# bkomuves/zikkurat-algebra

Hardware: AMD Instinct MI355X
Metric: BLS12-381 G1 MSM pairs/sec at 2^20; Fr NTT 2^24 elems/sec (1/2/4/8 GPU) (higher is better)
Workload: dtype u32-limb Montgomery Fp (381-bit)

## Files before the change

include/zkalgebra_gpu.h:

```cpp
#ifndef ZKALGEBRA_GPU_H
#define ZKALGEBRA_GPU_H

#include <stddef.h>
#include <stdint.h>

#ifdef __cplusplus
extern "C" {
#endif

#define ZKG_API __attribute__((visibility("default")))


ZKG_API void bn128_G1_proj_MSM_mont_coeff_proj_out(int npoints, const uint64_t *expos, const uint64_t *grps, uint64_t *tgt, int expo_nlimbs);
ZKG_API void bn128_G1_proj_MSM_std_coeff_proj_out(int npoints, const uint64_t *expos, const uint64_t *grps, uint64_t *tgt, int expo_nlimbs);
ZKG_API void bn128_G1_proj_MSM_mont_coeff_affine_out(int npoints, const uint64_t *expos, const uint64_t *grps, uint64_t *tgt, int expo_nlimbs);
ZKG_API void bn128_G1_proj_MSM_std_coeff_affine_out(int npoints, const uint64_t *expos, const uint64_t *grps, uint64_t *tgt, int expo_nlimbs);
ZKG_API void bn128_G1_proj_MSM_std_coeff_proj_out_variable(int npoints, const uint64_t *expos, const uint64_t *grps, uint64_t *tgt, int expo_nlimbs, int window_size);

ZKG_API void bls12_381_G1_proj_MSM_mont_coeff_proj_out(int npoints, const uint64_t *expos, const uint64_t *grps, uint64_t *tgt, int expo_nlimbs);
ZKG_API void bls12_381_G1_proj_MSM_std_coeff_proj_out(int npoints, const uint64_t *expos, const uint64_t *grps, uint64_t *tgt, int expo_nlimbs);
ZKG_API void bls12_381_G1_proj_MSM_mont_coeff_affine_out(int npoints, const uint64_t *expos, const uint64_t *grps, uint64_t *tgt, int expo_nlimbs);
ZKG_API void bls12_381_G1_proj_MSM_std_coeff_affine_out(int npoints, const uint64_t *expos, const uint64_t *grps, uint64_t *tgt, int expo_nlimbs);
ZKG_API void bls12_381_G1_proj_MSM_std_coeff_proj_out_variable(int npoints, const uint64_t *expos, const uint64_t *grps, uint64_t *tgt, int expo_nlimbs, int window_size);

// ... 271 lines not shown
                                     const uint64_t *base_affine, int affine_out, uint64_t *d_tgt);
ZKG_API int zkg_g2_scl_powers(int curve, int n, const uint64_t *a, const uint64_t *tau, const uint64_t *base_affine,
                              int affine_out, uint64_t *tgt);
ZKG_API void zkg_g2_scl_set_window(int c);
ZKG_API void zkg_g2_scl_set_fixed_min(int n);
ZKG_API int  zkg_g2_scl_last_path(void);
ZKG_API size_t zkg_g2_scl_table_bytes(int curve, int c);

ZKG_API void zkg_g1_proj_add(int curve, const uint64_t *a, const uint64_t *b, uint64_t *out);
ZKG_API void zkg_g1_proj_normalize(int curve, const uint64_t *a, uint64_t *out);
ZKG_API void zkg_g1_proj_to_affine(int curve, const uint64_t *a, uint64_t *out);

ZKG_API void zkg_gen_fr(int curve, uint64_t seed, int64_t start, int64_t count, uint64_t *out);
ZKG_API void zkg_gen_g1_points(int curve, uint64_t seed, int64_t start, int64_t count, uint64_t *out);
ZKG_API void zkg_fft_generator(int curve, int m, uint64_t *out);

ZKG_API int zkg_msm_default_window(int npoints);
ZKG_API int zkg_msm_window(int curve, int npoints, int expo_nlimbs, int expos_mont);

ZKG_API void zkg_msm_profile(int on);
ZKG_API void zkg_msm_set_group_limit(size_t entries);
ZKG_API void zkg_msm_set_ysum_mode(int mode);
ZKG_API void zkg_msm_set_ahead_min(int lg);
ZKG_API void zkg_ntt_set_max_radix(int r);
ZKG_API void zkg_ntt_set_table_max(size_t entries);
ZKG_API void zkg_ntt_ext_set_max_grid(unsigned tiles);
ZKG_API void zkg_ntt_set_cache_limit(size_t bytes);
ZKG_API size_t zkg_ntt_cache_bytes(void);
ZKG_API void zkg_arena_set_limit(size_t bytes);
ZKG_API int zkg_msm_last_groups(void);
ZKG_API int zkg_g1_fft_last_glv(void);
ZKG_API int zkg_g1_fft_plan(int curve, int m, int *bits, int cap);
ZKG_API int zkg_g1_fft_radix_products(int b);
ZKG_API size_t zkg_msm_workspace_bytes(int curve, int npoints, int expo_nlimbs, int expos_mont, int host_inputs,
                                       int window_size, int groups);

ZKG_API void bn128_pairing_affine(const uint64_t *P, const uint64_t *Q, uint64_t *tgt);
ZKG_API void bn128_pairing_projective(const uint64_t *P, const uint64_t *Q, uint64_t *tgt);
ZKG_API void bls12_381_pairing_affine(const uint64_t *P, const uint64_t *Q, uint64_t *tgt);
ZKG_API void bls12_381_pairing_projective(const uint64_t *P, const uint64_t *Q, uint64_t *tgt);
ZKG_API int zkg_pairing_rows(int curve, int n, const uint64_t *P, const uint64_t *Q, uint64_t *tgt);
ZKG_API int zkg_pairing_rows_device(int curve, int n, const uint64_t *d_P, const uint64_t *d_Q, uint64_t *d_tgt);
ZKG_API int zkg_pairing_product(int curve, int n, const uint64_t *P, const uint64_t *Q, uint64_t *tgt);
ZKG_API int zkg_pairing_product_device(int curve, int n, const uint64_t *d_P, const uint64_t *d_Q, uint64_t *d_tgt);
ZKG_API int zkg_pairing_final_expo(int curve, int n, const uint64_t *src, uint64_t *tgt);
ZKG_API int zkg_pairing_final_expo_device(int curve, int n, const uint64_t *d_src, uint64_t *d_tgt);
// ... 24 lines not shown
```

zikkurat-algebra_amd/csrc/zk_capi.cpp:

```cpp
#include <hip/hip_runtime.h>
#include <string.h>
#include "../../include/zkalgebra_gpu.h"
#include "zk_gen.hpp"
#include "zk_host.hpp"
#include "zk_msm.hpp"
#include "zk_ntt.hpp"
#include "zk_runtime.hpp"

using namespace zk;

namespace {

enum Out { PROJ, AFFINE, JAC };

template <class C>
void msm_entry(int npoints, const uint64_t *expos, const uint64_t *grps, uint64_t *tgt, int nl, bool mont,
               int window, Out out) {
  using HF = typename HostOf<C>::Fp;
  constexpr int NP = C::NP64;
  uint64_t proj[3 * NP];
  bool ok = false;
  guard([&] {
    msm_g1<C>(npoints, expos, nl, grps, true, mont, window, proj);
    ok = true;
// ... 318 lines not shown
    const uint64_t v[] = ZK_BN128_FFT_GEN_FR64;
    memcpy(g.v, v, sizeof g.v);
    for (int i = m; i < ZK_BN128_FFT_LOG; i++) zkh::sqr(g, g);
    memcpy(out, g.v, sizeof g.v);
  } else {
    zkh::Fe<zkh::BLS_Fr> g;
    const uint64_t v[] = ZK_BLS12_381_FFT_GEN_FR64;
    memcpy(g.v, v, sizeof g.v);
    for (int i = m; i < ZK_BLS12_381_FFT_LOG; i++) zkh::sqr(g, g);
    memcpy(out, g.v, sizeof g.v);
  }
}

ZKG_API int zkg_msm_default_window(int npoints) { return zk::msm_default_window(npoints); }
ZKG_API int zkg_msm_window(int curve, int npoints, int expo_nlimbs, int expos_mont) {
  const int bits = expos_mont ? (curve == ZKG_BN128 ? 254 : 255) : 64 * (expo_nlimbs < 4 ? expo_nlimbs : 4);
  return zk::msm_default_window_bits(npoints, bits);
}

ZKG_API void zkg_msm_profile(int on) { zk::msm_set_profile(on); }
ZKG_API void zkg_msm_set_group_limit(size_t entries) { zk::msm_set_group_limit(entries); }
ZKG_API void zkg_msm_set_ysum_mode(int mode) { zk::msm_set_ysum_mode(mode); }
ZKG_API void zkg_msm_set_ahead_min(int lg) { zk::msm_set_ahead_min(lg); }
ZKG_API void zkg_ntt_set_max_radix(int r) { zk::ntt_set_max_radix(r); }

ZKG_API void zkg_ntt_set_table_max(size_t entries) { zk::ntt_set_table_max(entries); }
ZKG_API void zkg_ntt_ext_set_max_grid(unsigned tiles) { zk::ntt_ext_set_max_grid(tiles); }
ZKG_API void zkg_ntt_set_cache_limit(size_t bytes) { zk::ntt_set_cache_limit(bytes); }
ZKG_API size_t zkg_ntt_cache_bytes(void) { return guard_ret<size_t>(0, [&] { return zk::ntt_cache_bytes(); }); }
ZKG_API void zkg_arena_set_limit(size_t bytes) { zk::arena_set_limit(bytes); }
ZKG_API int zkg_msm_last_groups(void) { return zk::msm_last_groups_read(); }
ZKG_API size_t zkg_msm_workspace_bytes(int curve, int npoints, int expo_nlimbs, int expos_mont, int host_inputs,
                                       int window_size, int groups) {
  return guard_ret<size_t>(0, [&] {
    if (curve == ZKG_BN128)
      return zk::msm_workspace_bytes<BN254>(npoints, expo_nlimbs, expos_mont != 0, host_inputs != 0, window_size,
                                            groups);
    return zk::msm_workspace_bytes<BLS381>(npoints, expo_nlimbs, expos_mont != 0, host_inputs != 0, window_size,
                                           groups);
  });
}

ZKG_API int zkg_set_devices(const int *ids, int n) { return zk::set_device_set(ids, n); }
ZKG_API int zkg_get_devices(int *ids, int cap) {
  const std::vector<int> v = zk::device_set();
  for (int i = 0; i < (int)v.size() && i < cap; i++) ids[i] = v[i];
// ... 24 lines not shown
```

zikkurat-algebra_amd/csrc/zk_msm.hip:

```cpp
#include "zk_msm_impl.hpp"

namespace zk {

int msm_default_window(int n) {
  if (n <= 1) return 4;
  const int lg = ilog2((unsigned)n);
  int c;
  if (lg <= 10) c = lg - 1;
  else if (lg <= 12) c = 10;
  else if (lg <= 16) c = 13;
  else if (lg <= 24) c = 16;
  else c = 20;
  if (c < 4) c = 4;
  if (c > 20) c = 20;
  return c;
}

int msm_default_window_bits(int n, int bits) {
  const int c = msm_default_window(n);
  if (n <= 1) return c;
  const int lg = ilog2((unsigned)n);
  if (bits == 254 && lg >= 20 && lg <= 24) return 17;
  if (bits == 255 && (lg == 23 || lg == 24)) return 20;
  return c;
}

void msm_set_ysum_mode(int mode) { ysum_mode().store(mode < 0 ? -1 : (mode ? 1 : 0)); }
void msm_set_ahead_min(int lg) { msm_ahead_min().store(lg < 0 ? -1 : lg); }
void msm_set_profile(int on) { msm_profile_flag().store(on); }
int msm_last_groups_read() { return msm_last_groups().load(); }
void msm_set_group_limit(size_t entries) {
  msm_group_limit().store(entries == 0 || entries > MSM_MAX_GROUP_ENTRIES ? MSM_MAX_GROUP_ENTRIES : entries);
}

template size_t msm_workspace_bytes<BN254>(int, int, bool, bool, int, int);
template size_t msm_workspace_bytes<BLS381>(int, int, bool, bool, int, int);
template void msm_g1<BN254>(int, const uint64_t *, int, const uint64_t *, bool, bool, int, uint64_t *);
template void msm_g1<BLS381>(int, const uint64_t *, int, const uint64_t *, bool, bool, int, uint64_t *);

}
```

zikkurat-algebra_amd/csrc/zk_msm.hpp:

```cpp
#pragma once
#include <stddef.h>
#include <stdint.h>
#include "zk_curve.hpp"
#include "zk_host.hpp"

namespace zk {

template <class C> struct HostOf;
template <> struct HostOf<BN254> {
  using Fp = zkh::BN_Fp;
  using Fr = zkh::BN_Fr;
  static void b3(zkh::Fe<Fp> &r) { const uint64_t v[] = ZK_BN128_B3_FP64; memcpy(r.v, v, sizeof r.v); }
};
template <> struct HostOf<BLS381> {
  using Fp = zkh::BLS_Fp;
  using Fr = zkh::BLS_Fr;
  static void b3(zkh::Fe<Fp> &r) { const uint64_t v[] = ZK_BLS12_381_B3_FP64; memcpy(r.v, v, sizeof r.v); }
};

template <> struct HostOf<BN254_G2> {
  using Fp = zkh::HF2<zkh::BN_Fp>;
  using Fr = zkh::BN_Fr;
};
template <> struct HostOf<BLS381_G2> {
  using Fp = zkh::HF2<zkh::BLS_Fp>;
  using Fr = zkh::BLS_Fr;
};

int msm_default_window(int n);
int msm_default_window_bits(int n, int bits);
void msm_set_profile(int on);
void msm_set_group_limit(size_t entries);
void msm_set_ysum_mode(int mode);
void msm_set_ahead_min(int lg);
int msm_last_groups_read();

template <class C>
size_t msm_workspace_bytes(int n, int nl, bool mont, bool host_inputs, int window, int groups);
template <class C>
void msm_g1(int n, const uint64_t *scalars, int nl, const uint64_t *points, bool host_inputs, bool mont,
            int window, uint64_t *out_proj);

}
```

zikkurat-algebra_amd/csrc/zk_msm_impl.hpp:

```cpp
#pragma once
#include <hipcub/hipcub.hpp>
#include <algorithm>
#include <atomic>
#include <chrono>
#include <memory>
#include <thread>
#include <vector>
#include "zk_curve.hpp"
#include "zk_quad.hpp"
#include "zk_host.hpp"
#include "zk_runtime.hpp"
#include "zk_msm.hpp"
#include "zk_ntt.hpp"

namespace zk {

template <class C>
__global__ void __launch_bounds__(256) k_points_int(const uint64_t *__restrict__ pts, int n,
                                                    uint32_t *__restrict__ out) {
  using F = typename C::Fp;
  constexpr int IN4 = 2 * F::N64 * 8 / 16;
  constexpr int OUT4 = aff_words<F>() / 4;
  constexpr int ST4 = IN4 > OUT4 ? IN4 : OUT4;
  __shared__ uint4 stage[256 * ST4];
// ... 85 lines not shown
constexpr int FINE_LDS_MAX = 8192;
constexpr int FINE_LDS_BYTES = 150 * 1024;
static int fine_stage_cap(int s) {
  const int cap = (FINE_LDS_BYTES - (4 << s)) / 4;
  return cap < FINE_LDS_MAX ? cap : FINE_LDS_MAX;
}

__device__ __forceinline__ uint32_t block_excl_scan256(uint32_t v, uint32_t *tmp, uint32_t *total) {
  const int t = threadIdx.x;
  tmp[t] = v;
  __syncthreads();
  for (int d = 1; d < 256; d <<= 1) {
    const uint32_t o = t >= d ? tmp[t - d] : 0;
    __syncthreads();
    tmp[t] += o;
    __syncthreads();
  }
  const uint32_t incl = tmp[t];
  *total = tmp[255];
  __syncthreads();
  return incl - v;
}

template <bool SCATTER>
__global__ void __launch_bounds__(256) k_coarse(const uint32_t *__restrict__ dig, int n, int plo, int phi, int M,
                                                int s, int nbins, uint32_t *__restrict__ cnt,
                                                uint32_t *__restrict__ tmpv, uint16_t *__restrict__ tmpf) {
  __shared__ uint32_t hist[MSM_COARSE_BINS], lofs[MSM_COARSE_BINS], gcur[MSM_COARSE_BINS], scan_tmp[256];
  __shared__ uint32_t sv[SORT_CHUNK], sk[SORT_CHUNK];
  const uint32_t w = blockIdx.y, g = blockIdx.x, nwg = gridDim.x;
  const int t = threadIdx.x;
  const int e0 = plo + (int)g * M, e1 = min(phi, e0 + M);
  const uint32_t *d = dig + (size_t)w * n;
  uint32_t *cw = cnt + (size_t)w * nbins * nwg + g;
  if (!SCATTER) {
    if (w == 0 && g == 0 && t == 0) cnt[(size_t)gridDim.y * nbins * nwg] = 0;
    for (int b = t; b < nbins; b += 256) hist[b] = 0;
    __syncthreads();
    for (int b0 = e0; b0 < e1; b0 += 256 * COUNT_ILP) {
      uint32_t mag[COUNT_ILP];
#pragma unroll
      for (int j = 0; j < COUNT_ILP; j++) {
        const int e = b0 + j * 256 + t;
        mag[j] = e < e1 ? d[e] & 0x7fffffffu : 0u;
      }
#pragma unroll
      for (int j = 0; j < COUNT_ILP; j++)
        if (mag[j]) atomicAdd(&hist[(mag[j] - 1) >> s], 1u);
    }
    __syncthreads();
    for (int b = t; b < nbins; b += 256) cw[(size_t)b * nwg] = hist[b];
    return;
  }
  for (int b = t; b < nbins; b += 256) gcur[b] = cw[(size_t)b * nwg];
  const uint32_t fmask = (1u << s) - 1;
  constexpr int PER = SORT_CHUNK / 256;
  for (int c0 = e0; c0 < e1; c0 += SORT_CHUNK) {
    for (int b = t; b < nbins; b += 256) hist[b] = 0;
    __syncthreads();
    uint32_t val[PER], key[PER], rank[PER];
#pragma unroll
    for (int k = 0; k < PER; k++) {
      const int e = c0 + k * 256 + t;
      const uint32_t v = e < e1 ? d[e] : 0u;
      const uint32_t mag = v & 0x7fffffffu;
      key[k] = 0xffffffffu;
      if (mag) {
        const uint32_t b = (mag - 1) >> s;
        key[k] = (b << 16) | ((mag - 1) & fmask);
        val[k] = (uint32_t)e | (v & 0x80000000u);
        rank[k] = atomicAdd(&hist[b], 1u);
      }
    }
    __syncthreads();
    uint32_t tot;
    const uint32_t h = t < nbins ? hist[t] : 0u;
    const uint32_t ex = block_excl_scan256(h, scan_tmp, &tot);
    if (t < nbins) lofs[t] = ex;
    __syncthreads();
#pragma unroll
    for (int k = 0; k < PER; k++) {
      if (key[k] != 0xffffffffu) {
        const uint32_t p = lofs[key[k] >> 16] + rank[k];
        sv[p] = val[k];
        sk[p] = key[k];
      }
    }
    __syncthreads();
    for (uint32_t i = t; i < tot; i += 256) {
      const uint32_t k = sk[i], b = k >> 16;
      const uint32_t slot = gcur[b] + (i - lofs[b]);
      tmpv[slot] = sv[i];
      tmpf[slot] = (uint16_t)(k & 0xffffu);
    }
    __syncthreads();
    if (t < nbins) gcur[t] += h;
  }
}

template <bool SCATTER>
// ... 85 lines not shown
    const int leader = __ffsll((unsigned long long)m) - 1;
    const uint32_t lk = (uint32_t)__builtin_amdgcn_readlane((int)key, leader);
    const bool mine = todo && key == lk;
    const uint64_t same = __ballot(mine);
    const int cnt = __popcll(same);
    if (cnt < 4) break;
    if (RET) {
      uint32_t base = 0;
      if ((int)lane == leader) base = atomicAdd(&ctr[lk], (uint32_t)cnt);
      base = (uint32_t)__builtin_amdgcn_readlane((int)base, leader);
      if (mine) r = base + (uint32_t)__popcll(same & below);
    } else if ((int)lane == leader) {
      atomicAdd(&ctr[lk], (uint32_t)cnt);
    }
    if (mine) todo = false;
  }
  if (todo) {
    if (RET) r = atomicAdd(&ctr[key], 1u);
    else atomicAdd(&ctr[key], 1u);
  }
  return r;
}

template <int BS>
__device__ __forceinline__ uint32_t block_excl_scan(uint32_t v, uint32_t *wtot, uint32_t *total) {
  const int t = threadIdx.x, lane = t & 63, w = t >> 6;
  uint32_t x = v;
#pragma unroll
  for (int d = 1; d < 64; d <<= 1) {
    const uint32_t o = (uint32_t)__shfl_up((int)x, d, 64);
    if (lane >= d) x += o;
  }
  if (lane == 63) wtot[w] = x;
  __syncthreads();
  uint32_t off = 0, all = 0;
#pragma unroll
  for (int k = 0; k < BS / 64; k++) {
    off += k < w ? wtot[k] : 0u;
    all += wtot[k];
  }
  *total = all;
  __syncthreads();
  return off + x - v;
}

template <int FINE_BS, int FINE_ILP, bool AGG>
static __global__ void __launch_bounds__(FINE_BS) k_fine(const uint32_t *__restrict__ coff, int nwg, uint32_t nq,
                                                         int s, int cap, const uint32_t *__restrict__ tmpv,
                                                         const uint16_t *__restrict__ tmpf,
                                                         uint32_t *__restrict__ list, uint32_t *__restrict__ offsets,
                                                         uint32_t base) {
  extern __shared__ uint32_t fh[];
  __shared__ uint32_t wtot[FINE_BS / 64];
  const int F = 1 << s, t = threadIdx.x;
  uint32_t *sv = fh + F;
  const uint32_t q = blockIdx.x;
  const uint32_t start = coff[(size_t)q * nwg];
  const uint32_t end = coff[(size_t)(q + 1) * nwg];
  const bool staged = end - start <= (uint32_t)cap;
  constexpr uint32_t STEP = FINE_BS * FINE_ILP;
  for (int f = t; f < F; f += FINE_BS) fh[f] = 0;
  __syncthreads();
  for (uint32_t e0 = start; e0 < end; e0 += STEP) {
    uint32_t k[FINE_ILP];
#pragma unroll
    for (int j = 0; j < FINE_ILP; j++) {
      const uint32_t e = e0 + j * FINE_BS + t;
      k[j] = e < end ? tmpf[e] : 0u;
    }
#pragma unroll
    for (int j = 0; j < FINE_ILP; j++) {
      const bool act = e0 + j * FINE_BS + t < end;
      if (AGG) lds_inc_agg<false>(fh, k[j], act);
      else if (act) atomicAdd(&fh[k[j]], 1u);
    }
  }
  __syncthreads();
  const int per = (F + FINE_BS - 1) / FINE_BS;
  uint32_t sum = 0;
  for (int j = 0; j < per; j++) {
    const int f = t * per + j;
    if (f < F) sum += fh[f];
  }
  uint32_t tot;
  uint32_t run = block_excl_scan<FINE_BS>(sum, wtot, &tot);
  for (int j = 0; j < per; j++) {
    const int f = t * per + j;
    if (f < F) {
      const uint32_t h = fh[f];
      fh[f] = staged ? run : start + run;
      offsets[(size_t)q * F + f] = base + start + run;
      run += h;
    }
  }
  if (q == nq - 1 && t == 0) offsets[(size_t)nq * F] = base + end;
  __syncthreads();
  for (uint32_t e0 = start; e0 < end; e0 += STEP) {
    uint32_t k[FINE_ILP], v[FINE_ILP];
#pragma unroll
    for (int j = 0; j < FINE_ILP; j++) {
      const uint32_t e = e0 + j * FINE_BS + t;
      k[j] = e < end ? tmpf[e] : 0u;
      v[j] = e < end ? tmpv[e] : 0u;
    }
#pragma unroll
    for (int j = 0; j < FINE_ILP; j++) {
      const bool act = e0 + j * FINE_BS + t < end;
      const uint32_t slot = AGG ? lds_inc_agg<true>(fh, k[j], act) : (act ? atomicAdd(&fh[k[j]], 1u) : 0u);
      if (act) {
        if (staged) sv[slot] = v[j];
        else list[slot] = v[j];
      }
    }
  }
  if (staged) {
    __syncthreads();
    for (uint32_t i = t; i < end - start; i += FINE_BS) list[start + i] = sv[i];
  }
}
// ... 6 lines not shown
  }
  return lo;
}

typedef __attribute__((address_space(3))) void lds_void_t;
typedef __attribute__((address_space(1))) void glb_void_t;

#ifndef ZK_ACCUM_WAVES14
#define ZK_ACCUM_WAVES14 2
#endif
#ifndef ZK_ACCUM_WAVES20
#define ZK_ACCUM_WAVES20 2
#endif
template <class F>
struct AccumOcc {
  static constexpr int waves = F::N >= 28 ? 1 : (F::N > 14 ? ZK_ACCUM_WAVES20 : (F::N == 14 ? ZK_ACCUM_WAVES14 : 3));
};

template <class C>
__global__ void __launch_bounds__(256, AccumOcc<typename C::Fp>::waves)
    k_accum(const uint32_t *__restrict__ points, const uint32_t *__restrict__ list,
            const uint32_t *__restrict__ offsets, uint32_t nb, int CH, uint32_t W, uint32_t B,
            uint32_t *__restrict__ buckets, uint32_t *__restrict__ ikeys, uint32_t *__restrict__ ivals,
            uint32_t nslots, const uint8_t *__restrict__ filled) {
  using F = typename C::Fp;
  constexpr int AW = aff_words<F>();
  constexpr int NCH = AW / 4;
  __shared__ uint4 stage[4][NCH][64];
  const int wave = threadIdx.x >> 6, lane = threadIdx.x & 63;
  const uint32_t t = blockIdx.x * blockDim.x + threadIdx.x;
  const uint32_t total = offsets[nb];
  const uint32_t cs = offsets[0] + t * (uint32_t)CH;
  const bool active = 2 * t < nslots && cs < total;
  uint32_t k0 = nb, k1 = nb;
  uint32_t tail_b = nb, tail_slot = 0;
  bool head_end = false;
  Xyzz<F> acc;
  xyzz_set_inf(acc);
  auto prefetch = [&](uint32_t c) {
    const uint32_t *src = points + (size_t)(c & 0x7fffffffu) * AW;
#pragma unroll
    for (int j = 0; j < NCH; j++)
      __builtin_amdgcn_global_load_lds((glb_void_t *)(src + 4 * j), (lds_void_t *)&stage[wave][j][0], 16, 0, 0);
  };
  auto read_point = [&](Aff<F> &P) {
    uint32_t w[AW];
#pragma unroll
    for (int j = 0; j < NCH; j++) {
      const uint4 v = stage[wave][j][lane];
      w[4 * j] = v.x; w[4 * j + 1] = v.y; w[4 * j + 2] = v.z; w[4 * j + 3] = v.w;
    }
#pragma unroll
    for (int i = 0; i < F::N; i++) {
      P.x.v[i] = w[i];
      P.y.v[i] = w[F::SN + i];
    }
  };
  auto start_run = [&](uint32_t b) {
    if (filled && filled[b]) xyzz_load(acc, buckets + (size_t)b * xyzz_words<F>());
    else xyzz_set_inf(acc);
  };
  if (active) {
    const uint32_t ce = min(total, cs + (uint32_t)CH);
    uint32_t b = bucket_of(offsets, nb, cs);
    uint32_t bbeg = offsets[b], bend = offsets[b + 1];
    if (bbeg >= cs) start_run(b);
    uint32_t bnext = offsets[min(b + 2, nb)];
    bool first_run = true;
    const uint32_t last = ce - 1;
    uint32_t c0 = list[cs], c1 = list[min(cs + 1, last)];
    prefetch(c0);
    for (uint32_t e = cs; e < ce; e++) {
      Aff<F> P;
      read_point(P);
      asm volatile("s_waitcnt lgkmcnt(0)" ::: "memory");
      prefetch(c1);
      const uint32_t c2 = list[min(e + 2, last)];
      if (e >= bend) {
        if (first_run && bbeg < cs) {
          xyzz_store(ivals + (size_t)(2 * t) * xyzz_words<F>(), acc);
          k0 = b;
        } else {
          xyzz_store(buckets + (size_t)b * xyzz_words<F>(), acc);
        }
        first_run = false;
        do {
          b++;
// ... 460 lines not shown
        Xyzz<F> o;
        xyzz_load(o, park + (size_t)t * XW);
        xyzz_add_red(acc, o);
      }
      __syncthreads();
    }
    if (t < S) {
      const int y = hiY ? (1 << l0) + seg : seg;
      xyzz_store(Y + ((size_t)w * NY + y) * XW, acc);
    }
  }
}

template <class C, int WAVES = 2>
__global__ void __launch_bounds__(256, WAVES) k_ysum3(const uint32_t *__restrict__ buckets,
                                                  const uint32_t *__restrict__ offsets,
                                                  const uint8_t *__restrict__ filled, int W, int c, int l0,
                                                  SegRegion r0, SegRegion r1, uint32_t *__restrict__ Y) {
  using F = typename C::Fp;
  constexpr int XW = xyzz_words<F>();
  constexpr int NCH = XW / 4;
  __shared__ uint4 stage[4][NCH][64];
  static_assert(4 * NCH * 64 * 16 >= 128 * XW * 4, "the fold's park area fits the prefetch image");
  uint32_t *park = reinterpret_cast<uint32_t *>(&stage[0][0][0]);
  const int l1 = c - 1 - l0;
  const int NY = (1 << l0) + (1 << l1);
  const int nb0 = r0.count * r0.G / 256, nb1 = r1.count * r1.G / 256;
  const int w = blockIdx.x / (nb0 + nb1);
  int rb = blockIdx.x % (nb0 + nb1);
  const bool hiY = rb < nb0;
  const SegRegion r = hiY ? r0 : r1;
  if (!hiY) rb -= nb0;
  const int G = r.G, S = 256 / G;
  const int t = threadIdx.x, wave = t >> 6, lane = t & 63;
  const int seg = rb * S + t % S, part = t / S;
  const int per = r.len / G;
  const uint32_t B = 1u << (c - 1);
  const uint32_t *wb = buckets + (size_t)w * B * XW;
  auto bucket_m = [&](int s) -> uint32_t {
    return hiY ? ((uint32_t)seg << l0) + (uint32_t)s : ((uint32_t)s << l0) + (uint32_t)seg;
  };
  auto nonempty = [&](uint32_t rank) -> bool {
    return filled ? filled[rank] != 0 : offsets[rank + 1] > offsets[rank];
  };
  auto prefetch = [&](uint32_t m) {
    const uint32_t *src = wb + (size_t)m * XW;
// ... 301 lines not shown
    const int lb = c - 1;
    s.fs = lb > 8 ? lb - 8 : 0;
    s.nbins = 1 << (lb - s.fs);
    size_t M = ((size_t)W * n + 2047) / 2048;
    M = (M + 255) & ~(size_t)255;
    s.M = (int)(M < 2048 ? 2048 : M);
    s.nwg = (int)(((size_t)s.nsplit_max() + s.M - 1) / s.M);
    static const bool split_on = [] {
      const char *e = getenv("ZK_SORT_SPLIT");
      return !(e && e[0] == '0');
    }();
    const size_t per_bin = (size_t)s.nsplit_max() / s.nbins;
    const size_t half_cap = (size_t)fine_stage_cap(s.fs) / 2;
    while (split_on && s.fs >= 10 && s.s2 < s.fs && s.s2 < 8 && (per_bin >> s.s2) > half_cap) s.s2++;
    if (s.s2) {
      const size_t w2 = per_bin / 16384;
      s.nwg2 = (int)(w2 < 1 ? 1 : (w2 > 64 ? 64 : w2));
    }
  }
  s.CH = s.split_ch(0);
  return s;
}

inline int MsmShape::split_ch(int h) const {
  const size_t ent = (size_t)W * (size_t)(split_lo(h + 1) - split_lo(h));
  const size_t ch = ent >> 17, lo = n > 4096 ? 8 : 4;
  int r = ch >= 64 ? 64 : (ch <= lo ? (int)lo : (int)ch);
  if (ent >= ((size_t)1 << 25)) r = 128;
  if (const char *e = getenv("ZK_MSM_CH")) {
    const int v = atoi(e);
    if (v > 0) r = v;
  }
  return r;
}

template <class F>
constexpr int stitch_bs() { return xyzz_words<F>() > 64 ? 128 : 256; }
template <class F>
constexpr int stitch_bs0() { return (ZK_STITCH_QUAD && is_base_field<F>()) ? STITCH_QBS : stitch_bs<F>(); }

static size_t stitch_slots0(const MsmShape &s) {
  size_t m = 0;
  for (int h = 0; h < s.NS; h++) {
    const size_t ch = (size_t)s.split_ch(h);
    m = std::max(m, 2 * (((size_t)s.W * (s.split_lo(h + 1) - s.split_lo(h)) + ch - 1) / ch));
  }
  return m;
// ... 13 lines not shown
  const size_t xw = xyzz_words<F>() * 4;
  const size_t nb = (size_t)s.W * s.B;
  const size_t maxent = (size_t)s.W * s.n;
  const size_t ns0 = stitch_slots0(s), ns1 = stitch_slots1(s, stitch_bs0<F>());
  size_t cub = 0, cub2 = 0;
  ZK_CHECK(hipcub::DeviceScan::ExclusiveSum(nullptr, cub, (uint32_t *)nullptr, (uint32_t *)nullptr, (int)(s.nmat() + 1)));
  ZK_CHECK(hipcub::DeviceScan::ExclusiveSum(nullptr, cub2, (uint32_t *)nullptr, (uint32_t *)nullptr, (int)ns0));
  if (s.s2) {
    size_t cub3 = 0;
    ZK_CHECK(hipcub::DeviceScan::ExclusiveSum(nullptr, cub3, (uint32_t *)nullptr, (uint32_t *)nullptr, (int)(s.nmat2() + 1)));
    if (cub3 > cub2) cub2 = cub3;
  }
  size_t bytes = 0;
  auto add = [&](size_t b) { bytes += (b + 255) & ~size_t(255); };
  add(maxent * 4 * 3);
  add(maxent * 2);
  add((s.nmat() + 1) * 4 * 2);
  if (s.s2) {
    add(maxent * 2);
    add((s.nmat2() + 1) * 4 * 2);
  }
  add(s.NS * (nb + 1) * 4);
  add(nb);
  add(ns0 * (xw + 4) + ns0 * 16 + 64);
  add(ns1 * (xw + 4) * 2);
  add(nb * xw);
  add((size_t)s.W * s.NY * xw);
  add(cub > cub2 ? cub : cub2);
  if (s.NS > 1) add(cub > cub2 ? cub : cub2);
  return bytes + (1 << 20);
}

inline std::atomic<int> &msm_last_groups() {
  static std::atomic<int> v{0};
  return v;
}

inline std::atomic<int> &msm_profile_flag() {
  static std::atomic<int> on{0};
  return on;
}
struct PhaseProf {
  bool on = false;
  hipStream_t st = nullptr;
  std::vector<std::pair<const char *, hipEvent_t>> ev;
  explicit PhaseProf(hipStream_t s) : st(s) {
// ... 27 lines not shown
  int stride, loff, nread;
  bool mont;
};

template <class C>
struct GroupPass {
  using F = typename C::Fp;
  static constexpr int STITCH_BS = stitch_bs<F>();
  Device &dev;
  MsmShape s;
  ScalarSlice sc;
  int wbase, timer_slot;
  const uint32_t *pts_int;
  uint64_t *h;
  PhaseProf *prof;
  hipStream_t st;
  size_t nb, xw, maxent, ns0, ns1, cub = 0;
  uint32_t *list, *dig, *tmpv, *cnt, *coff, *offsets, *ikeys0, *ivals0, *ckeys, *cidx, *flags, *pos, *ccount;
  uint16_t *tmpf, *tmpf2 = nullptr;
  uint32_t *cnt2 = nullptr, *coff2 = nullptr;
  uint32_t *okA, *ovA, *okB, *ovB, *buckets, *Y;
  void *cubtmp;
  uint8_t *filled = nullptr;
  hipStream_t sst = nullptr;
  void *cubtmp_sort = nullptr;
  const uint64_t *pts_ref = nullptr;
  std::vector<hipEvent_t> sorted_ev;
  hipEvent_t presorted = nullptr;
  const uint32_t *inK, *inV;
  size_t slots;
  uint32_t *outK, *outV, *altK, *altV;

  GroupPass(Device &d, const MsmShape &shape, const ScalarSlice &scal, int wb, const uint32_t *pts, uint64_t *hh,
            PhaseProf *pr, hipStream_t stream, int tslot)
      : dev(d), s(shape), sc(scal), wbase(wb), timer_slot(tslot), pts_int(pts), h(hh), prof(pr), st(stream) {
    const int n = s.n;
    nb = (size_t)s.W * s.B;
    xw = xyzz_words<F>();
    maxent = (size_t)s.W * n;
    ZK_REQUIRE(maxent <= MSM_MAX_PASS_ENTRIES, "msm: window group exceeds the sort capacity (internal sizing bug)");
    list = dev.arena.take<uint32_t>(maxent);
    dig = dev.arena.take<uint32_t>(maxent);
    tmpv = dev.arena.take<uint32_t>(maxent);
    tmpf = dev.arena.take<uint16_t>(maxent);
    cnt = dev.arena.take<uint32_t>(s.nmat() + 1);
    coff = dev.arena.take<uint32_t>(s.nmat() + 1);
    if (s.s2) {
      tmpf2 = dev.arena.take<uint16_t>(maxent);
      cnt2 = dev.arena.take<uint32_t>(s.nmat2() + 1);
      coff2 = dev.arena.take<uint32_t>(s.nmat2() + 1);
    }
    offsets = dev.arena.take<uint32_t>((size_t)s.NS * (nb + 1));
    if (s.NS > 1) filled = dev.arena.take<uint8_t>(nb);
    ns0 = stitch_slots0(s);
    ns1 = stitch_slots1(s, stitch_bs0<F>());
    ikeys0 = dev.arena.take<uint32_t>(ns0);
    ivals0 = dev.arena.take<uint32_t>(ns0 * xw);
    ckeys = dev.arena.take<uint32_t>(ns0);
    cidx = dev.arena.take<uint32_t>(ns0);
    flags = dev.arena.take<uint32_t>(ns0);
    pos = dev.arena.take<uint32_t>(ns0);
    ccount = dev.arena.take<uint32_t>(16);
    okA = dev.arena.take<uint32_t>(ns1);
    ovA = dev.arena.take<uint32_t>(ns1 * xw);
    okB = dev.arena.take<uint32_t>(ns1);
    ovB = dev.arena.take<uint32_t>(ns1 * xw);
    buckets = dev.arena.take<uint32_t>(nb * xw);
    Y = dev.arena.take<uint32_t>((size_t)s.W * s.NY * xw);
    size_t cub2 = 0;
    ZK_CHECK(hipcub::DeviceScan::ExclusiveSum(nullptr, cub, cnt, coff, (int)(s.nmat() + 1), st));
    ZK_CHECK(hipcub::DeviceScan::ExclusiveSum(nullptr, cub2, flags, pos, (int)ns0, st));
    if (cub2 > cub) cub = cub2;
    if (s.s2) {
      size_t cub3 = 0;
      ZK_CHECK(hipcub::DeviceScan::ExclusiveSum(nullptr, cub3, cnt2, coff2, (int)(s.nmat2() + 1), st));
      if (cub3 > cub) cub = cub3;
    }
    cubtmp = dev.arena.take<char>(cub);
// ... 24 lines not shown
    const uint16_t *ff = tmpf + base;
    int fnwg = s.nwg, fs = s.fs;
    uint32_t nq = (uint32_t)(s.W * s.nbins);
    if (s.s2) {
      const int nsub = 1 << s.s2, s2sh = s.fs - s.s2;
      const dim3 g2((unsigned)s.nwg2, nq);
      hipLaunchKernelGGL(k_split<false>, g2, dim3(256), 0, st, coff, s.nwg, s2sh, nsub, cnt2, tmpv + base, tmpf + base,
                         dig + base, tmpf2 + base);
      ZK_CHECK(hipGetLastError());
      size_t cb2 = cub;
      ZK_CHECK(hipcub::DeviceScan::ExclusiveSum(cubtmp, cb2, cnt2, coff2, (int)(s.nmat2() + 1), st));
      hipLaunchKernelGGL(k_split<true>, g2, dim3(256), 0, st, coff, s.nwg, s2sh, nsub, coff2, tmpv + base, tmpf + base,
                         dig + base, tmpf2 + base);
      ZK_CHECK(hipGetLastError());
      fv = dig + base;
      ff = tmpf2 + base;
      fcoff = coff2;
      fnwg = s.nwg2;
      fs = s2sh;
      nq *= (uint32_t)nsub;
    }
    const int cap = fine_stage_cap(fs);
    const int lds = (4 << fs) + 4 * cap;
    if ((size_t)(hi - lo) * s.W >= (size_t)nq * 4096) {
      ZK_CHECK(hipFuncSetAttribute((const void *)k_fine<1024, 4, true>, hipFuncAttributeMaxDynamicSharedMemorySize,
                                   lds));
      hipLaunchKernelGGL((k_fine<1024, 4, true>), dim3(nq), dim3(1024), lds, st, fcoff, fnwg, nq, fs, cap, fv, ff,
                         list + base, offsets + (size_t)sp * (nb + 1), base);
    } else {
      ZK_CHECK(hipFuncSetAttribute((const void *)k_fine<256, 1, false>, hipFuncAttributeMaxDynamicSharedMemorySize,
                                   lds));
      hipLaunchKernelGGL((k_fine<256, 1, false>), dim3(nq), dim3(256), lds, st, fcoff, fnwg, nq, fs, cap, fv, ff,
                         list + base, offsets + (size_t)sp * (nb + 1), base);
    }
    ZK_CHECK(hipGetLastError());
    if (st == this->st) mark("sort");
  }

  std::vector<hipEvent_t> wait_sc, wait_pt;
  const std::atomic<int> *ready_sc = nullptr, *ready_pt = nullptr;
  void wait_for(hipStream_t on, const std::vector<hipEvent_t> &ev, const std::atomic<int> *ready, int sp) {
    if (sp >= (int)ev.size() || !ev[sp]) return;
    if (ready)
      while (!ready[sp].load(std::memory_order_acquire)) std::this_thread::yield();
    ZK_CHECK(hipStreamWaitEvent(on, ev[sp], 0));
  }
  void convert(int sp) {
    const int lo = s.split_lo(sp), hi = s.split_lo(sp + 1);
    if (hi <= lo) return;
    hipLaunchKernelGGL(k_points_int<C>, dim3(div_up(hi - lo, 256)), dim3(256), 0, st,
                       pts_ref + (size_t)lo * 2 * C::NP64, hi - lo, const_cast<uint32_t *>(pts_int) + (size_t)lo * aff_words<F>());
    ZK_CHECK(hipGetLastError());
  }
  int ch0 = 0;
  void accumulate(int sp) {
    if (sp == 0) timer_begin(dev, timer_slot, st);
    const size_t npts = (size_t)s.split_lo(sp + 1) - (size_t)s.split_lo(sp);
    const int CH = s.split_ch(sp);
    ch0 = CH;
    const size_t nsl = 2 * (((size_t)s.W * npts + CH - 1) / CH);
    hipLaunchKernelGGL(k_accum<C>, dim3(div_up(nsl / 2, 256)), dim3(256), 0, st, pts_int, list,
                       offsets + (size_t)sp * (nb + 1), (uint32_t)nb, CH, (uint32_t)s.W, (uint32_t)s.B, buckets,
                       ikeys0, ivals0, (uint32_t)nsl, (const uint8_t *)(sp > 0 ? filled : nullptr));
    ZK_CHECK(hipGetLastError());
    if (sp == s.NS - 1) timer_end(dev, timer_slot, st);
    mark("accum");
    inK = ikeys0;
    inV = ivals0;
    slots = nsl;
    level = 0;
    outK = okA; outV = ovA; altK = okB; altV = ovB;
  }
  void fill_mark(int sp) {
    hipLaunchKernelGGL(k_fill_mark, dim3(div_up(nb, 256)), dim3(256), 0, st, offsets + (size_t)sp * (nb + 1),
                       (uint32_t)nb, sp == 0 ? 1 : 0, filled);
    ZK_CHECK(hipGetLastError());
  }

  int level = 0;
  bool stitch_level() {
    const bool raw = ZK_STITCH_RAW && level++ > 0;
    const bool quad0 = stitch_bs0<F>() == STITCH_QBS && (ns0 <= 65536 || ch0 >= 64);
    const int bs = raw ? STITCH_BS : (quad0 ? STITCH_QBS : STITCH_BS);
    const bool final_level = slots <= (size_t)bs;
    const size_t nout = final_level ? 2 : 2 * ((slots + bs - 1) / bs);
    if (raw) {
// ... 501 lines not shown
```

zikkurat-algebra_amd/zkalgebra.py:

```python
import ctypes
import os
from dataclasses import dataclass

import numpy as np

HERE = os.path.dirname(os.path.abspath(__file__))
LIB_PATH = os.environ.get("ZK_LIB_PATH") or os.path.join(HERE, "lib", "libzkalgebra_gpu.so")
U64P = ctypes.POINTER(ctypes.c_uint64)

CURVES = ("bn128", "bls12_381")
CURVE_ID = {"bn128": 0, "bls12_381": 1}
NLIMBS_P = {"bn128": 4, "bls12_381": 6}
NLIMBS_R = 4
FFT_LOG = {"bn128": 28, "bls12_381": 32}

REFERENCE_SYMBOLS = [
    f"{c}_G1_proj_MSM_{k}_coeff_{o}_out" for c in CURVES for k in ("mont", "std") for o in ("proj", "affine")
] + [f"{c}_G1_proj_MSM_std_coeff_proj_out_variable" for c in CURVES] + [
    f"{c}_G1_jac_MSM_{k}_coeff_{o}_out" for c in CURVES for k in ("mont", "std") for o in ("jac", "affine")
] + [f"{c}_poly_mont_ntt_{d}" for c in CURVES for d in ("forward", "inverse")]
ARR_OPS = ["is_valid", "is_zero", "is_one", "is_equal", "set_zero", "set_one", "set_const", "copy", "from_std",
           "to_std", "append", "neg", "add", "sub", "sqr", "mul", "inv", "div", "neg_inplace", "add_inplace",
           "sub_inplace", "sqr_inplace", "mul_inplace", "inv_inplace", "div_inplace", "sub_inplace_reverse",
           "mul_add", "mul_sub", "dot_prod", "powers", "scale", "scale_inplace", "Ax_plus_y", "Ax_plus_y_inplace",
           "Ax_plus_By", "Ax_plus_By_inplace"]
REFERENCE_SYMBOLS += [f"{c}_arr_mont_{o}" for c in CURVES for o in ARR_OPS] + [
    f"{c}_poly_mont_{k}_by_vanishing" for c in CURVES for k in ("div", "quot")] + [
    f"{c}_G1_{co}_{f}" for c in CURVES for co in ("proj", "jac")
    for f in ("batch_from_affine", "batch_to_affine", "fft_forward", "fft_inverse")] + [
    f"{c}_G2_proj_MSM_{k}_coeff_{o}_out" for c in CURVES for k in ("mont", "std") for o in ("proj", "affine")] + [
    f"{c}_G2_proj_{f}" for c in CURVES
    for f in ("batch_from_affine", "batch_to_affine", "MSM_std_coeff_proj_out_variable")] + [
    f"{c}_G2_proj_fft_{d}" for c in CURVES for d in ("forward", "inverse")]
EXTENSION_SYMBOLS = [
    "zkg_version", "zkg_device_count", "zkg_set_device", "zkg_device_malloc", "zkg_device_free",
    "zkg_memcpy_htod", "zkg_memcpy_dtoh", "zkg_device_synchronize", "zkg_g1_msm_device", "zkg_ntt_device",
    "zkg_g1_proj_add", "zkg_g1_proj_normalize", "zkg_g1_proj_to_affine", "zkg_gen_fr", "zkg_gen_g1_points",
    "zkg_fft_generator", "zkg_msm_default_window", "zkg_msm_window", "zkg_timer_enable", "zkg_timer_reset", "zkg_timer_read",
    "zkg_arr_op_device", "zkg_arr_dot_device", "zkg_arr_powers_device",
    "zkg_poly_div_by_vanishing_device", "zkg_g1_fft_device", "zkg_g1_batch_to_affine_device",
    "zkg_g1_jac_fft_device", "zkg_g1_jac_batch_to_affine_device", "zkg_g2_msm_device",
    "zkg_msm_profile", "zkg_msm_set_group_limit", "zkg_msm_set_ysum_mode", "zkg_msm_set_ahead_min", "zkg_ntt_set_max_radix", "zkg_ntt_set_table_max",
    "zkg_arena_set_limit", "zkg_msm_last_groups", "zkg_g1_fft_last_glv", "zkg_g1_fft_plan", "zkg_g1_fft_radix_products", "zkg_msm_workspace_bytes", "zkg_set_devices", "zkg_get_devices",
    "zkg_release", "zkg_comm_unique_id", "zkg_comm_init", "zkg_comm_destroy", "zkg_comm_rank", "zkg_comm_world",
    "zkg_comm_allgather", "zkg_comm_barrier", "zkg_comm_max_f64", "zkg_g1_comm_sum_partials",
    "zkg_g1_msm_device_sharded", "zkg_set_error_mode", "zkg_last_error", "zkg_g2_batch_to_affine_device",
    "zkg_g2_fft_device", "zkg_g2_fft_set_max_lanes",
]

POLY_OPS = ["degree", "is_zero", "is_equal", "neg", "add", "sub", "scale", "lincomb", "mul_naive", "eval_at"]
REFERENCE_SYMBOLS += [f"{c}_poly_mont_{o}" for c in CURVES for o in POLY_OPS]
EXTENSION_SYMBOLS += ["zkg_poly_mul_device", "zkg_poly_eval_device", "zkg_poly_lincomb_device",
                      "zkg_poly_set_mul_direct_max", "zkg_poly_last_mul_path"]
POLY_MUL_MAX_LOG = {"bn128": 28, "bls12_381": 30}
EXTENSION_SYMBOLS += ["zkg_poly_long_div_device", "zkg_poly_long_div", "zkg_poly_set_div_base_max",
                      "zkg_poly_div_base_max", "zkg_poly_div_plan", "zkg_poly_last_div_steps",
                      "zkg_poly_div_profile", "zkg_poly_last_div_phase_ms"]
EXTENSION_SYMBOLS += ["zkg_ntt_ext_device", "zkg_ntt_ext", "zkg_ntt_ext_set_max_grid"]
EXTENSION_SYMBOLS += ["zkg_ntt_set_cache_limit", "zkg_ntt_cache_bytes"]
EXTENSION_SYMBOLS += [f"zkg_g1_scl_{k}{d}" for k in ("fixed", "rows", "powers") for d in ("", "_device")] + [
    "zkg_g1_scl_set_window", "zkg_g1_scl_set_fixed_min", "zkg_g1_scl_last_path", "zkg_g1_scl_digits",
    "zkg_g1_scl_table_bytes"]
EXTENSION_SYMBOLS += [f"zkg_g2_scl_{k}{d}" for k in ("fixed", "rows", "powers") for d in ("", "_device")] + [
    "zkg_g2_scl_set_window", "zkg_g2_scl_set_fixed_min", "zkg_g2_scl_last_path", "zkg_g2_scl_table_bytes"]
REFERENCE_SYMBOLS += [f"{c}_pairing_{k}" for c in CURVES for k in ("affine", "projective")]
# ... 818 lines not shown
                             window)
    return out


def g2_msm_device(curve, n, d_scalars, d_points, mont=True, window=0, nlimbs=4):
    out = np.zeros(6 * NLIMBS_P[curve], dtype=np.uint64)
    load().zkg_g2_msm_device(CURVE_ID[curve], n, d_scalars.ptr, nlimbs, 1 if mont else 0, d_points.ptr, _p(out),
                             window)
    return out


def msm_profile(on):
    load().zkg_msm_profile(1 if on else 0)


def msm_set_ysum_mode(mode):
    load().zkg_msm_set_ysum_mode(int(mode))


def msm_set_ahead_min(lg):
    load().zkg_msm_set_ahead_min(int(lg))


def msm_set_group_limit(entries):
    load().zkg_msm_set_group_limit(int(entries))


def ntt_set_max_radix(r):
    load().zkg_ntt_set_max_radix(int(r))


def arr_op_device(curve, op, n, d_a, d_b=None, d_c=None, kA=None, kB=None, d_tgt=None):
    z = np.zeros(4, dtype=np.uint64)
    ka = np.ascontiguousarray(kA if kA is not None else z, dtype=np.uint64)
    kb = np.ascontiguousarray(kB if kB is not None else z, dtype=np.uint64)
    load().zkg_arr_op_device(CURVE_ID[curve], ARR_OP_CODE[op], n, d_a.ptr if d_a else None,
                             d_b.ptr if d_b else None, d_c.ptr if d_c else None, _p(ka), _p(kb), d_tgt.ptr)


def arr_dot_device(curve, n, d_a, d_b):
    out = np.zeros(4, dtype=np.uint64)
    load().zkg_arr_dot_device(CURVE_ID[curve], n, d_a.ptr, d_b.ptr, _p(out))
    return out


def arr_powers_device(curve, n, kA, kB, d_tgt):
# ... 743 lines not shown
```

Measured before the change: 326.7 million.

## Precompute per-chunk starting bucket in fine sort instead of binary search in accum

New measurement: 327.5 million (median of 5 runs). No clear change (+0.3%).

```diff
diff --git a/include/zkalgebra_gpu.h b/include/zkalgebra_gpu.h
--- a/include/zkalgebra_gpu.h
+++ b/include/zkalgebra_gpu.h
@@ -317,6 +317,7 @@
 ZKG_API void zkg_msm_set_group_limit(size_t entries);
 ZKG_API void zkg_msm_set_ysum_mode(int mode);
 ZKG_API void zkg_msm_set_ahead_min(int lg);
+ZKG_API void zkg_msm_set_chunk(int ch);
 ZKG_API void zkg_ntt_set_max_radix(int r);
 ZKG_API void zkg_ntt_set_table_max(size_t entries);
 ZKG_API void zkg_ntt_ext_set_max_grid(unsigned tiles);
diff --git a/zikkurat-algebra_amd/csrc/zk_capi.cpp b/zikkurat-algebra_amd/csrc/zk_capi.cpp
--- a/zikkurat-algebra_amd/csrc/zk_capi.cpp
+++ b/zikkurat-algebra_amd/csrc/zk_capi.cpp
@@ -364,6 +364,7 @@
 ZKG_API void zkg_msm_set_group_limit(size_t entries) { zk::msm_set_group_limit(entries); }
 ZKG_API void zkg_msm_set_ysum_mode(int mode) { zk::msm_set_ysum_mode(mode); }
 ZKG_API void zkg_msm_set_ahead_min(int lg) { zk::msm_set_ahead_min(lg); }
+ZKG_API void zkg_msm_set_chunk(int ch) { zk::msm_set_chunk(ch); }
 ZKG_API void zkg_ntt_set_max_radix(int r) { zk::ntt_set_max_radix(r); }
 
 ZKG_API void zkg_ntt_set_table_max(size_t entries) { zk::ntt_set_table_max(entries); }
diff --git a/zikkurat-algebra_amd/csrc/zk_msm.hip b/zikkurat-algebra_amd/csrc/zk_msm.hip
--- a/zikkurat-algebra_amd/csrc/zk_msm.hip
+++ b/zikkurat-algebra_amd/csrc/zk_msm.hip
@@ -27,6 +27,7 @@
 
 void msm_set_ysum_mode(int mode) { ysum_mode().store(mode < 0 ? -1 : (mode ? 1 : 0)); }
 void msm_set_ahead_min(int lg) { msm_ahead_min().store(lg < 0 ? -1 : lg); }
+void msm_set_chunk(int ch) { msm_chunk_force().store(ch <= 0 ? 0 : (ch < 4 ? 4 : (ch > 1024 ? 1024 : ch))); }
 void msm_set_profile(int on) { msm_profile_flag().store(on); }
 int msm_last_groups_read() { return msm_last_groups().load(); }
 void msm_set_group_limit(size_t entries) {
diff --git a/zikkurat-algebra_amd/csrc/zk_msm.hpp b/zikkurat-algebra_amd/csrc/zk_msm.hpp
--- a/zikkurat-algebra_amd/csrc/zk_msm.hpp
+++ b/zikkurat-algebra_amd/csrc/zk_msm.hpp
@@ -33,6 +33,7 @@
 void msm_set_group_limit(size_t entries);
 void msm_set_ysum_mode(int mode);
 void msm_set_ahead_min(int lg);
+void msm_set_chunk(int ch);
 int msm_last_groups_read();
 
 template <class C>
diff --git a/zikkurat-algebra_amd/csrc/zk_msm_impl.hpp b/zikkurat-algebra_amd/csrc/zk_msm_impl.hpp
--- a/zikkurat-algebra_amd/csrc/zk_msm_impl.hpp
+++ b/zikkurat-algebra_amd/csrc/zk_msm_impl.hpp
@@ -131,6 +131,28 @@
   return incl - v;
 }
 
+template <int BS>
+__device__ __forceinline__ uint32_t block_excl_scan(uint32_t v, uint32_t *wtot, uint32_t *total) {
+  const int t = threadIdx.x, lane = t & 63, w = t >> 6;
+  uint32_t x = v;
+#pragma unroll
+  for (int d = 1; d < 64; d <<= 1) {
+    const uint32_t o = (uint32_t)__shfl_up((int)x, d, 64);
+    if (lane >= d) x += o;
+  }
+  if (lane == 63) wtot[w] = x;
+  __syncthreads();
+  uint32_t off = 0, all = 0;
+#pragma unroll
+  for (int k = 0; k < BS / 64; k++) {
+    off += k < w ? wtot[k] : 0u;
+    all += wtot[k];
+  }
+  *total = all;
+  __syncthreads();
+  return off + x - v;
+}
+
 template <bool SCATTER>
 __global__ void __launch_bounds__(256) k_coarse(const uint32_t *__restrict__ dig, int n, int plo, int phi, int M,
                                                 int s, int nbins, uint32_t *__restrict__ cnt,
@@ -171,8 +193,12 @@
 #pragma unroll
     for (int k = 0; k < PER; k++) {
       const int e = c0 + k * 256 + t;
-      const uint32_t v = e < e1 ? d[e] : 0u;
-      const uint32_t mag = v & 0x7fffffffu;
+      val[k] = e < e1 ? d[e] : 0u;
+    }
+#pragma unroll
+    for (int k = 0; k < PER; k++) {
+      const int e = c0 + k * 256 + t;
+      const uint32_t v = val[k], mag = v & 0x7fffffffu;
       key[k] = 0xffffffffu;
       if (mag) {
         const uint32_t b = (mag - 1) >> s;
@@ -184,7 +210,7 @@
     __syncthreads();
     uint32_t tot;
     const uint32_t h = t < nbins ? hist[t] : 0u;
-    const uint32_t ex = block_excl_scan256(h, scan_tmp, &tot);
+    const uint32_t ex = block_excl_scan<256>(h, scan_tmp, &tot);
     if (t < nbins) lofs[t] = ex;
     __syncthreads();
 #pragma unroll
@@ -316,36 +342,18 @@
   return r;
 }
 
-template <int BS>
-__device__ __forceinline__ uint32_t block_excl_scan(uint32_t v, uint32_t *wtot, uint32_t *total) {
-  const int t = threadIdx.x, lane = t & 63, w = t >> 6;
-  uint32_t x = v;
-#pragma unroll
-  for (int d = 1; d < 64; d <<= 1) {
-    const uint32_t o = (uint32_t)__shfl_up((int)x, d, 64);
-    if (lane >= d) x += o;
-  }
-  if (lane == 63) wtot[w] = x;
-  __syncthreads();
-  uint32_t off = 0, all = 0;
-#pragma unroll
-  for (int k = 0; k < BS / 64; k++) {
-    off += k < w ? wtot[k] : 0u;
-    all += wtot[k];
-  }
-  *total = all;
-  __syncthreads();
-  return off + x - v;
-}
-
+constexpr uint32_t FINE_LONG_RUN = 32;
+constexpr int FINE_LONG_MAX = 32;
 template <int FINE_BS, int FINE_ILP, bool AGG>
 static __global__ void __launch_bounds__(FINE_BS) k_fine(const uint32_t *__restrict__ coff, int nwg, uint32_t nq,
                                                          int s, int cap, const uint32_t *__restrict__ tmpv,
                                                          const uint16_t *__restrict__ tmpf,
                                                          uint32_t *__restrict__ list, uint32_t *__restrict__ offsets,
-                                                         uint32_t base) {
+                                                         uint32_t base, uint32_t *__restrict__ chunk_b, uint32_t CH,
+                                                         uint32_t nch) {
   extern __shared__ uint32_t fh[];
   __shared__ uint32_t wtot[FINE_BS / 64];
+  __shared__ uint32_t longrun[FINE_LONG_MAX][3], nlong;
   const int F = 1 << s, t = threadIdx.x;
   uint32_t *sv = fh + F;
   const uint32_t q = blockIdx.x;
@@ -354,6 +362,7 @@
   const bool staged = end - start <= (uint32_t)cap;
   constexpr uint32_t STEP = FINE_BS * FINE_ILP;
   for (int f = t; f < F; f += FINE_BS) fh[f] = 0;
+  if (t == 0) nlong = 0;
   __syncthreads();
   for (uint32_t e0 = start; e0 < end; e0 += STEP) {
     uint32_t k[FINE_ILP];
@@ -384,11 +393,31 @@
       const uint32_t h = fh[f];
       fh[f] = staged ? run : start + run;
       offsets[(size_t)q * F + f] = base + start + run;
+      if (h) {
+        const uint32_t beg = start + run, bkt = q * (uint32_t)F + (uint32_t)f;
+        const uint32_t c0 = (beg + CH - 1) / CH, c1 = min(nch, (beg + h + CH - 1) / CH);
+        uint32_t slot = FINE_LONG_MAX;
+        if (c1 > c0 + FINE_LONG_RUN) slot = atomicAdd(&nlong, 1u);
+        if (slot < (uint32_t)FINE_LONG_MAX) {
+          longrun[slot][0] = bkt;
+          longrun[slot][1] = c0;
+          longrun[slot][2] = c1;
+        } else {
+          for (uint32_t k = c0; k < c1; k++) chunk_b[k] = bkt;
+        }
+      }
       run += h;
     }
   }
   if (q == nq - 1 && t == 0) offsets[(size_t)nq * F] = base + end;
   __syncthreads();
+  {
+    const uint32_t nl = min(nlong, (uint32_t)FINE_LONG_MAX);
+    for (uint32_t i = 0; i < nl; i++) {
+      const uint32_t bkt = longrun[i][0], c1 = longrun[i][2];
+      for (uint32_t k = longrun[i][1] + t; k < c1; k += FINE_BS) chunk_b[k] = bkt;
+    }
+  }
   for (uint32_t e0 = start; e0 < end; e0 += STEP) {
     uint32_t k[FINE_ILP], v[FINE_ILP];
 #pragma unroll
@@ -441,7 +470,7 @@
     k_accum(const uint32_t *__restrict__ points, const uint32_t *__restrict__ list,
             const uint32_t *__restrict__ offsets, uint32_t nb, int CH, uint32_t W, uint32_t B,
             uint32_t *__restrict__ buckets, uint32_t *__restrict__ ikeys, uint32_t *__restrict__ ivals,
-            uint32_t nslots, const uint8_t *__restrict__ filled) {
+            uint32_t nslots, const uint8_t *__restrict__ filled, const uint32_t *__restrict__ chunk_b) {
   using F = typename C::Fp;
   constexpr int AW = aff_words<F>();
   constexpr int NCH = AW / 4;
@@ -481,7 +510,7 @@
   };
   if (active) {
     const uint32_t ce = min(total, cs + (uint32_t)CH);
-    uint32_t b = bucket_of(offsets, nb, cs);
+    uint32_t b = chunk_b[t];
     uint32_t bbeg = offsets[b], bend = offsets[b + 1];
     if (bbeg >= cs) start_run(b);
     uint32_t bnext = offsets[min(b + 2, nb)];
@@ -988,6 +1017,8 @@
   constexpr int NCH = XW / 4;
   __shared__ uint4 stage[4][NCH][64];
   static_assert(4 * NCH * 64 * 16 >= 128 * XW * 4, "the fold's park area fits the prefetch image");
+  static_assert(sizeof(uint4) * 4 * NCH * 64 <= 160 * 1024, "the prefetch image fits gfx950's 160 KB of LDS per CU");
+  static_assert(is_base_field<F>() || WAVES == 1, "an Fp2 image (> 64 KB) leaves room for one block per CU only");
   uint32_t *park = reinterpret_cast<uint32_t *>(&stage[0][0][0]);
   const int l1 = c - 1 - l0;
   const int NY = (1 << l0) + (1 << l1);
@@ -1335,7 +1366,12 @@
   return s;
 }
 
+inline std::atomic<int> &msm_chunk_force() {
+  static std::atomic<int> v{0};
+  return v;
+}
 inline int MsmShape::split_ch(int h) const {
+  if (const int f = msm_chunk_force().load()) return f;
   const size_t ent = (size_t)W * (size_t)(split_lo(h + 1) - split_lo(h));
   const size_t ch = ent >> 17, lo = n > 4096 ? 8 : 4;
   int r = ch >= 64 ? 64 : (ch <= lo ? (int)lo : (int)ch);
@@ -1395,6 +1431,7 @@
   }
   add(s.NS * (nb + 1) * 4);
   add(nb);
+  add(s.NS * (ns0 / 2) * 4);
   add(ns0 * (xw + 4) + ns0 * 16 + 64);
   add(ns1 * (xw + 4) * 2);
   add(nb * xw);
@@ -1468,6 +1505,7 @@
   uint32_t *okA, *ovA, *okB, *ovB, *buckets, *Y;
   void *cubtmp;
   uint8_t *filled = nullptr;
+  uint32_t *chunkb = nullptr;
   hipStream_t sst = nullptr;
   void *cubtmp_sort = nullptr;
   const uint64_t *pts_ref = nullptr;
@@ -1500,6 +1538,7 @@
     if (s.NS > 1) filled = dev.arena.take<uint8_t>(nb);
     ns0 = stitch_slots0(s);
     ns1 = stitch_slots1(s, stitch_bs0<F>());
+    chunkb = dev.arena.take<uint32_t>((size_t)s.NS * (ns0 / 2));
     ikeys0 = dev.arena.take<uint32_t>(ns0);
     ivals0 = dev.arena.take<uint32_t>(ns0 * xw);
     ckeys = dev.arena.take<uint32_t>(ns0);
@@ -1570,16 +1609,19 @@
     }
     const int cap = fine_stage_cap(fs);
     const int lds = (4 << fs) + 4 * cap;
+    const uint32_t CH = (uint32_t)s.split_ch(sp);
+    const uint32_t nch = (uint32_t)(((size_t)s.W * (hi - lo) + CH - 1) / CH);
+    uint32_t *heads = chunkb + (size_t)sp * (ns0 / 2);
     if ((size_t)(hi - lo) * s.W >= (size_t)nq * 4096) {
       ZK_CHECK(hipFuncSetAttribute((const void *)k_fine<1024, 4, true>, hipFuncAttributeMaxDynamicSharedMemorySize,
                                    lds));
       hipLaunchKernelGGL((k_fine<1024, 4, true>), dim3(nq), dim3(1024), lds, st, fcoff, fnwg, nq, fs, cap, fv, ff,
-                         list + base, offsets + (size_t)sp * (nb + 1), base);
+                         list + base, offsets + (size_t)sp * (nb + 1), base, heads, CH, nch);
     } else {
       ZK_CHECK(hipFuncSetAttribute((const void *)k_fine<256, 1, false>, hipFuncAttributeMaxDynamicSharedMemorySize,
                                    lds));
       hipLaunchKernelGGL((k_fine<256, 1, false>), dim3(nq), dim3(256), lds, st, fcoff, fnwg, nq, fs, cap, fv, ff,
-                         list + base, offsets + (size_t)sp * (nb + 1), base);
+                         list + base, offsets + (size_t)sp * (nb + 1), base, heads, CH, nch);
     }
     ZK_CHECK(hipGetLastError());
     if (st == this->st) mark("sort");
@@ -1609,7 +1651,8 @@
     const size_t nsl = 2 * (((size_t)s.W * npts + CH - 1) / CH);
     hipLaunchKernelGGL(k_accum<C>, dim3(div_up(nsl / 2, 256)), dim3(256), 0, st, pts_int, list,
                        offsets + (size_t)sp * (nb + 1), (uint32_t)nb, CH, (uint32_t)s.W, (uint32_t)s.B, buckets,
-                       ikeys0, ivals0, (uint32_t)nsl, (const uint8_t *)(sp > 0 ? filled : nullptr));
+                       ikeys0, ivals0, (uint32_t)nsl, (const uint8_t *)(sp > 0 ? filled : nullptr),
+                       (const uint32_t *)(chunkb + (size_t)sp * (ns0 / 2)));
     ZK_CHECK(hipGetLastError());
     if (sp == s.NS - 1) timer_end(dev, timer_slot, st);
     mark("accum");
diff --git a/zikkurat-algebra_amd/zkalgebra.py b/zikkurat-algebra_amd/zkalgebra.py
--- a/zikkurat-algebra_amd/zkalgebra.py
+++ b/zikkurat-algebra_amd/zkalgebra.py
@@ -40,7 +40,7 @@
     "zkg_arr_op_device", "zkg_arr_dot_device", "zkg_arr_powers_device",
     "zkg_poly_div_by_vanishing_device", "zkg_g1_fft_device", "zkg_g1_batch_to_affine_device",
     "zkg_g1_jac_fft_device", "zkg_g1_jac_batch_to_affine_device", "zkg_g2_msm_device",
-    "zkg_msm_profile", "zkg_msm_set_group_limit", "zkg_msm_set_ysum_mode", "zkg_msm_set_ahead_min", "zkg_ntt_set_max_radix", "zkg_ntt_set_table_max",
+    "zkg_msm_profile", "zkg_msm_set_group_limit", "zkg_msm_set_ysum_mode", "zkg_msm_set_ahead_min", "zkg_msm_set_chunk", "zkg_ntt_set_max_radix", "zkg_ntt_set_table_max",
     "zkg_arena_set_limit", "zkg_msm_last_groups", "zkg_g1_fft_last_glv", "zkg_g1_fft_plan", "zkg_g1_fft_radix_products", "zkg_msm_workspace_bytes", "zkg_set_devices", "zkg_get_devices",
     "zkg_release", "zkg_comm_unique_id", "zkg_comm_init", "zkg_comm_destroy", "zkg_comm_rank", "zkg_comm_world",
     "zkg_comm_allgather", "zkg_comm_barrier", "zkg_comm_max_f64", "zkg_g1_comm_sum_partials",
@@ -905,6 +905,10 @@
     load().zkg_msm_set_ahead_min(int(lg))
 
 
+def msm_set_chunk(ch):
+    load().zkg_msm_set_chunk(int(ch))
+
+
 def msm_set_group_limit(entries):
     load().zkg_msm_set_group_limit(int(entries))
 
```
